# MITIBMxGraph/SALIENT_plusplus

Hardware: AMD Instinct MI355X
Metric: sampled_edges_per_sec (higher is better)
Workload: dtype int64/fp16-copy

## Files before the change

### include/spp.h

```cpp
#ifndef SPP_H
#define SPP_H

#include <stddef.h>
#include <stdint.h>

#ifdef __cplusplus
extern "C" {
#endif

#define SPP_ABI_VERSION 6
#define SPP_MAX_HOPS 8
#define SPP_MAX_PARTS 64

typedef int spp_status;
enum {
  SPP_OK = 0,
  SPP_ERR_INVALID = -1,
  SPP_ERR_HIP = -2,
  SPP_ERR_CAPACITY = -3,
  SPP_ERR_STATE = -4
};

int spp_abi_version(void);
const char* spp_last_error(void);
// ... 426 lines not shown
  int32_t reserved2;
  uint64_t seed;
} spp_agg_bwd_desc;

spp_status spp_agg_forward(const spp_agg_fwd_desc* desc, void* stream);
spp_status spp_agg_backward(const spp_agg_bwd_desc* desc, void* workspace_dev, int64_t workspace_bytes, void* stream);

spp_status spp_gather_rows_fp8(const void* q_dev, int64_t src_rows, int64_t F, const int8_t* scale_log2_dev,
                               const int64_t* idx_dev, int64_t n, void* dst_dev, void* stream);
spp_status spp_agg_forward_fp8(const spp_agg_fwd_desc* desc, const int8_t* scale_log2_dev, void* stream);

typedef struct spp_graph_agg_desc {
  int32_t epilogue;
  int32_t x_elem;
  int32_t out_elem;
  int32_t reserved;
  const int64_t* rowptr_dev;
  const int64_t* col_dev;
  const void* x_dev;
  int64_t x_stride_elems;
  int64_t x_rows;
  int64_t F;
  int64_t target_row0;
  const int64_t* target_ids_dev;
  int64_t num_targets;
  void* out_dev;
  int64_t out_stride_elems;
  float self_scale;
  int32_t reserved2;
} spp_graph_agg_desc;

int64_t spp_graph_agg_chunk(void);
int64_t spp_graph_agg_workspace_bytes(int64_t num_targets);
spp_status spp_graph_agg_forward(const spp_graph_agg_desc* desc, void* workspace_dev, int64_t workspace_bytes,
                                 void* stream);

#define SPP_GRAPH_AGG_MAX_PARTS 16
typedef struct spp_graph_agg_parts_desc {
  int32_t epilogue;
  int32_t x_elem;
  int32_t out_elem;
  int32_t num_parts;
  const int64_t* rowptr_dev;
  const int64_t* col_dev;
  int64_t part_offsets[SPP_GRAPH_AGG_MAX_PARTS + 1];
  const void* x_parts_dev[SPP_GRAPH_AGG_MAX_PARTS];
  int64_t x_stride_elems;
  int64_t F;
  int64_t target_row0;
  const int64_t* target_ids_dev;
  int64_t num_targets;
  void* out_dev;
  int64_t out_stride_elems;
  float self_scale;
  int32_t reserved;
} spp_graph_agg_parts_desc;

spp_status spp_graph_agg_parts_forward(const spp_graph_agg_parts_desc* desc, void* workspace_dev,
                                       int64_t workspace_bytes, void* stream);

typedef struct spp_graph_gat_desc {
  int32_t x_elem;
  int32_t out_elem;
  int32_t heads;
  int32_t relu;
  const int64_t* rowptr_dev;
  const int64_t* col_dev;
  const void* x_dev;
  int64_t x_stride_elems;
  int64_t x_rows;
  int64_t F;
  const float* a_src_dev;
  const float* a_dst_dev;
  int64_t target_row0;
  const int64_t* target_ids_dev;
  int64_t num_targets;
  void* out_dev;
  int64_t out_stride_elems;
  float negative_slope;
  int32_t reserved;
} spp_graph_gat_desc;

int64_t spp_graph_gat_chunk(void);
int64_t spp_graph_gat_workspace_bytes(int64_t num_targets);
spp_status spp_graph_gat_forward(const spp_graph_gat_desc* desc, void* workspace_dev, int64_t workspace_bytes,
                                 void* stream);

typedef struct spp_graph_gat_parts_desc {
  int32_t x_elem;
  int32_t out_elem;
  int32_t heads;
  int32_t relu;
  int32_t num_parts;
  int32_t reserved;
  const int64_t* rowptr_dev;
  const int64_t* col_dev;
  int64_t part_offsets[SPP_GRAPH_AGG_MAX_PARTS + 1];
  const void* h_parts_dev[SPP_GRAPH_AGG_MAX_PARTS];
  const float* a_parts_dev[SPP_GRAPH_AGG_MAX_PARTS];
  int64_t x_stride_elems;
  int64_t a_stride_elems;
  int64_t F;
  int64_t target_row0;
  const int64_t* target_ids_dev;
  int64_t num_targets;
  void* out_dev;
  int64_t out_stride_elems;
  float negative_slope;
  int32_t reserved2;
} spp_graph_gat_parts_desc;

spp_status spp_graph_gat_parts_forward(const spp_graph_gat_parts_desc* desc, void* workspace_dev,
                                       int64_t workspace_bytes, void* stream);

typedef struct spp_resinc_epilogue_desc {
  int32_t z_elem;
  int32_t r_elem;
  int32_t out_elem;
  float negative_slope;
  const void* z_dev;
  int64_t z_stride_elems;
  const float* a_dev;
  const float* b_dev;
  const void* r_dev;
  int64_t r_stride_elems;
  int64_t r_rows;
  int64_t r_row0;
  const int64_t* r_ids_dev;
  int64_t n;
  int64_t C;
  void* out_dev;
  int64_t out_stride_elems;
} spp_resinc_epilogue_desc;

spp_status spp_resinc_epilogue(const spp_resinc_epilogue_desc* desc, void* stream);

typedef struct spp_classify_desc {
  int32_t z_elem;
  int32_t reserved;
  const void* z_dev;
  int64_t z_stride_elems;
  int64_t n;
  int64_t C;
  const int64_t* y_dev;
  int64_t y_rows;
  int64_t y_row0;
  const int64_t* row_ids_dev;
  int64_t* pred_dev;
  float* nll_dev;
} spp_classify_desc;

spp_status spp_classify_rows(const spp_classify_desc* desc, void* stream);

#ifdef __cplusplus
}
#endif
#endif
```

### salient_plusplus_amd/_native.py

```python
import ctypes as C
import os

_HERE = os.path.dirname(os.path.abspath(__file__))
LIB_PATH = os.path.join(_HERE, "libspp_hip.so")

SPP_MAX_HOPS = 8
SPP_MAX_PARTS = 64

p = C.c_void_p
i32 = C.c_int32
i64 = C.c_int64
u32 = C.c_uint32


class PartitionCfg(C.Structure):
    _fields_ = [("num_parts", i32), ("rank", i32), ("offsets", i64 * (SPP_MAX_PARTS + 1)),
                ("use_cache", i32), ("cache_map_dev", p), ("cache_map_len", i64)]


class SamplerOpts(C.Structure):
    _fields_ = [("col32", i32), ("deg_tags", i32), ("row_stubs", i32), ("rng_arena", i32), ("rng_arena_mb", i64),
                ("fuse_scatter", i32), ("flag_tiled", i32), ("rows_coalesced", i32), ("dedup_preread", i32),
                ("fuse_max_edges", i64), ("initial_edge_cap", i64), ("reserved", i64 * 4)]


class SamplerCfg(C.Structure):
    _fields_ = [("rowptr_dev", p), ("col_dev", p), ("num_nodes", i64), ("nnz", i64),
                ("num_hops", i32), ("sizes", i64 * SPP_MAX_HOPS), ("max_batch", i64),
                ("num_slots", i32), ("device", i32), ("replace", i32), ("part", PartitionCfg),
                ("graph_generation", i64), ("opts", SamplerOpts)]


class SamplerInfo(C.Structure):
    _fields_ = [("col32", i32), ("deg_tags", i32), ("row_stubs", i32), ("rng_arena", i32), ("idbits", i32),
                ("tag_cap", i32), ("num_hops", i32), ("dedup_buckets_log2", i32), ("dedup_table_slots", i32),
                ("generic", i32 * SPP_MAX_HOPS), ("fused_pick", i32 * SPP_MAX_HOPS), ("flag_tiled", i32 * SPP_MAX_HOPS),
                ("rows_coalesced", i32 * SPP_MAX_HOPS), ("bucket_log2", i32 * SPP_MAX_HOPS),
                ("col32_ms", C.c_double), ("row_stubs_ms", C.c_double), ("rng_arena_ms", C.c_double),
                ("col32_bytes", i64), ("row_stubs_bytes", i64), ("rng_arena_bytes", i64), ("rng_arena_batches", i64)]


class MfgCounts(C.Structure):
    _fields_ = [("num_nodes", i64), ("num_seeds", i64), ("num_hops", i32),
                ("T", i64 * SPP_MAX_HOPS), ("S", i64 * SPP_MAX_HOPS), ("E", i64 * SPP_MAX_HOPS),
                ("draws", i64), ("part_counts", i64 * (SPP_MAX_PARTS + 2))]


class MfgOut(C.Structure):
    _fields_ = [("n_id", p), ("rowptr", p * SPP_MAX_HOPS), ("col", p * SPP_MAX_HOPS),
                ("parts", p), ("cached", p), ("perm", p), ("row_addr", p), ("x_remote", p)]


SPP_ELEM_F32, SPP_ELEM_F16, SPP_ELEM_BF16 = 0, 1, 2
SPP_ELEM_FP8_E4M3 = 3
SPP_AGG_DENSE, SPP_AGG_TABLE, SPP_AGG_ROWS = 0, 1, 2
SPP_AGG_MEAN, SPP_AGG_OPERAND, SPP_AGG_OPERAND_ACT, SPP_AGG_SUM = 0, 1, 2, 3
SPP_AGG_SCATTER, SPP_AGG_GATHER = 0, 1


class AggFwdDesc(C.Structure):
    _fields_ = [("source", i32), ("epilogue", i32), ("x_elem", i32), ("out_elem", i32), ("rowptr_dev", p),
                ("col_dev", p), ("num_targets", i64), ("x_dev", p), ("x_stride_elems", i64), ("x_rows", i64),
                ("n_id_dev", p), ("F", i64), ("out_dev", p), ("out_stride_elems", i64), ("self_scale", C.c_float),
                ("p", C.c_float), ("training", i32), ("reserved", i32), ("seed", C.c_uint64)]


class AggBwdDesc(C.Structure):
    _fields_ = [("form", i32), ("epilogue", i32), ("grad_elem", i32), ("out_elem", i32), ("z_elem", i32),
                ("reserved", i32), ("rowptr_dev", p), ("col_dev", p), ("num_targets", i64), ("num_sources", i64),
                ("num_edges", i64), ("grad_out_dev", p), ("grad_out_stride_elems", i64), ("F", i64),
                ("grad_x_dev", p), ("z_dev", p), ("self_scale", C.c_float), ("p", C.c_float), ("training", i32),
                ("reserved2", i32), ("seed", C.c_uint64)]


class GraphAggDesc(C.Structure):
    _fields_ = [("epilogue", i32), ("x_elem", i32), ("out_elem", i32), ("reserved", i32), ("rowptr_dev", p),
                ("col_dev", p), ("x_dev", p), ("x_stride_elems", i64), ("x_rows", i64), ("F", i64),
                ("target_row0", i64), ("target_ids_dev", p), ("num_targets", i64), ("out_dev", p),
                ("out_stride_elems", i64), ("self_scale", C.c_float), ("reserved2", i32)]


SPP_GRAPH_AGG_MAX_PARTS = 16


class GraphAggPartsDesc(C.Structure):
    _fields_ = [("epilogue", i32), ("x_elem", i32), ("out_elem", i32), ("num_parts", i32), ("rowptr_dev", p),
                ("col_dev", p), ("part_offsets", i64 * (SPP_GRAPH_AGG_MAX_PARTS + 1)),
                ("x_parts_dev", p * SPP_GRAPH_AGG_MAX_PARTS), ("x_stride_elems", i64), ("F", i64), ("target_row0", i64),
                ("target_ids_dev", p), ("num_targets", i64), ("out_dev", p), ("out_stride_elems", i64),
                ("self_scale", C.c_float), ("reserved", i32)]


class GraphGatDesc(C.Structure):
    _fields_ = [("x_elem", i32), ("out_elem", i32), ("heads", i32), ("relu", i32), ("rowptr_dev", p), ("col_dev", p),
                ("x_dev", p), ("x_stride_elems", i64), ("x_rows", i64), ("F", i64), ("a_src_dev", p), ("a_dst_dev", p),
                ("target_row0", i64), ("target_ids_dev", p), ("num_targets", i64), ("out_dev", p),
                ("out_stride_elems", i64), ("negative_slope", C.c_float), ("reserved", i32)]


class GraphGatPartsDesc(C.Structure):
    _fields_ = [("x_elem", i32), ("out_elem", i32), ("heads", i32), ("relu", i32), ("num_parts", i32), ("reserved", i32),
                ("rowptr_dev", p), ("col_dev", p), ("part_offsets", i64 * (SPP_GRAPH_AGG_MAX_PARTS + 1)),
                ("h_parts_dev", p * SPP_GRAPH_AGG_MAX_PARTS), ("a_parts_dev", p * SPP_GRAPH_AGG_MAX_PARTS),
                ("x_stride_elems", i64), ("a_stride_elems", i64), ("F", i64), ("target_row0", i64), ("target_ids_dev", p),
                ("num_targets", i64), ("out_dev", p), ("out_stride_elems", i64), ("negative_slope", C.c_float),
                ("reserved2", i32)]


class ResincEpilogueDesc(C.Structure):
    _fields_ = [("z_elem", i32), ("r_elem", i32), ("out_elem", i32), ("negative_slope", C.c_float), ("z_dev", p),
                ("z_stride_elems", i64), ("a_dev", p), ("b_dev", p), ("r_dev", p), ("r_stride_elems", i64),
                ("r_rows", i64), ("r_row0", i64), ("r_ids_dev", p), ("n", i64), ("C", i64), ("out_dev", p),
                ("out_stride_elems", i64)]


class ClassifyDesc(C.Structure):
    _fields_ = [("z_elem", i32), ("reserved", i32), ("z_dev", p), ("z_stride_elems", i64), ("n", i64), ("C", i64),
                ("y_dev", p), ("y_rows", i64), ("y_row0", i64), ("row_ids_dev", p), ("pred_dev", p), ("nll_dev", p)]


class GroupOut(C.Structure):
    _fields_ = [("mfg", MfgOut), ("x_out", p), ("y_out", p)]


class ExchangeCfg(C.Structure):
    _fields_ = [("comm", p), ("x_local_dev", p), ("x_local_rows", i64), ("row_bytes", i64),
                ("cache_feats_dev", p), ("cache_rows", i64), ("x_local_stride_bytes", i64),
                ("cache_stride_bytes", i64), ("peer_x_dev", C.POINTER(p)), ("peer_x_stride_bytes", i64),
                ("issue_on_consumer", i32),
                ("x_elem", i32), ("scale_log2_dev", p), ("scales_tag", C.c_uint64)]


class SessionCfg(C.Structure):
    _fields_ = [("rowptr_dev", p), ("col_dev", p), ("num_nodes", i64), ("nnz", i64),
                ("idx_dev", p), ("n_idx", i64), ("batch_size", i64), ("num_hops", i32),
                ("sizes", i64 * SPP_MAX_HOPS), ("skip_nonfull_batch", i32),
                ("force_exact_num_batches", i32), ("exact_num_batches", i64),
                ("max_items_in_queue", i32), ("group_size", i32), ("device", i32), ("sampler", p),
                ("part", C.POINTER(PartitionCfg)), ("exchange", C.POINTER(ExchangeCfg)),
                ("input_stream", p), ("order_after_input_stream", i32)]


class BatchDesc(C.Structure):
    _fields_ = [("batch_index", i64), ("start", i32), ("stop", i32), ("slot", i32),
                ("counts", MfgCounts)]


SIGNATURES = {
    "spp_abi_version": (C.c_int, []),
    "spp_last_error": (C.c_char_p, []),
    "spp_device_count": (C.c_int, []),
    "spp_async_errors": (C.c_int, [C.c_int, C.c_int]),
    "spp_profile_enable": (None, [C.c_int]),
    "spp_tune": (C.c_int, [C.c_char_p, C.c_int]),
    "spp_profile_read": (C.c_int, [C.c_int, C.POINTER(C.c_double), C.POINTER(i64), C.POINTER(i64)]),
    "spp_mt19937_fill": (C.c_int, [u32, i64, i64, p, p]),
    "spp_batch_seed": (u32, [i32]),
    "spp_gather_rows": (C.c_int, [p, i64, i64, p, C.c_int, i64, i64, p, p]),
    "spp_gather_rows_strided": (C.c_int, [p, i64, i64, i64, p, C.c_int, i64, i64, p, p]),
    "spp_to_row_major": (C.c_int, [p, i64, i64, C.c_int, p, p]),
    "spp_sampler_create": (C.c_int, [C.POINTER(SamplerCfg), C.POINTER(p)]),
    "spp_sampler_destroy": (None, [p]),
    "spp_sampler_workspace_bytes": (i64, [p]),
    "spp_sampler_deliver_stream": (p, [p]),
    "spp_sampler_get_cfg": (C.c_int, [p, C.POINTER(SamplerCfg)]),
    "spp_sampler_get_info": (C.c_int, [p, C.POINTER(SamplerInfo)]),
    "spp_sampler_sample": (C.c_int, [p, i32, p, i64, u32, i64, p]),
    "spp_sampler_wait": (C.c_int, [p, i32, C.POINTER(MfgCounts)]),
    "spp_sampler_export": (C.c_int, [p, i32, C.POINTER(MfgOut), p]),
    "spp_sampler_gather": (C.c_int, [p, i32, p, i64, i64, i64, i64, p, p]),
    "spp_nid2partid": (C.c_int, [p, i32, p, i64, p, p]),
    "spp_cache_build_map": (C.c_int, [p, i64, p, i64, p]),
    "spp_cache_lookup": (C.c_int, [p, i64, p, i64, p, p, p]),
    "spp_partition_workspace_bytes": (i64, [i64]),
    "spp_partition_batch": (C.c_int, [p, i64, p, i32, i32, i32, p, i64, i64, p, p, p, p, p, p, i64, p]),
    "spp_assemble_features": (C.c_int, [p, p, i64, p, i32, i32, i64, p, i64, p, p, p, i64, i64, i64, p, p, p]),
    "spp_session_create": (C.c_int, [C.POINTER(SessionCfg), C.POINTER(p)]),
    "spp_session_destroy": (None, [p]),
    "spp_session_num_total_batches": (i64, [p]),
    "spp_session_num_consumed_batches": (i64, [p]),
    "spp_session_batch_ranges": (C.c_int, [p, p]),
    "spp_session_next": (C.c_int, [p, C.POINTER(BatchDesc)]),
    "spp_session_export": (C.c_int, [p, C.POINTER(MfgOut), p, i64, i64, i64, p, p, i64, i64, p, p]),
    "spp_session_next_group": (C.c_int, [p, i32, C.POINTER(BatchDesc), C.POINTER(i32)]),
    "spp_session_export_group": (C.c_int, [p, i32, C.POINTER(GroupOut), p, i64, i64, i64, p, i64, i64, p]),
    "spp_session_blocked_us": (i64, [p]),
    "spp_session_blocked_occasions": (i64, [p]),
    "spp_session_sampler": (p, [p]),
    "spp_session_group_size": (i32, [p]),
    "spp_comm_unique_id": (C.c_int, [p]),
    "spp_comm_create": (C.c_int, [p, i32, i32, i32, C.POINTER(p)]),
    "spp_comm_create_local": (C.c_int, [i32, i32, C.POINTER(p)]),
    "spp_comm_destroy": (None, [p]),
    "spp_comm_rank": (i32, [p]),
    "spp_comm_world": (i32, [p]),
    "spp_vip_frequencies": (C.c_int, [p, p, i64, p, i64, i64, p, i32, p, p, p]),
    "spp_csr_mean_forward": (C.c_int, [p, p, i64, p, i32, i64, i64, p, i64, p]),
    "spp_csr_mean_backward": (C.c_int, [p, p, i64, p, i64, i64, p, p]),
    "spp_sage_operand_forward": (C.c_int, [p, p, i64, p, i32, i64, i64, p, i64, p]),
    "spp_sage_operand_forward_table": (C.c_int, [p, p, i64, p, i32, i64, i64, p, i64, p, i64, p]),
    "spp_sage_operand_backward": (C.c_int, [p, p, i64, i64, p, i64, i64, p, p]),
    "spp_sage_operand_backward_workspace_bytes": (i64, [i64, i64, i64]),
    "spp_sage_operand_backward_gather": (C.c_int, [p, p, i64, i64, i64, p, i64, i64, p, p, i64, p]),
    "spp_relu_dropout_forward": (C.c_int, [p, i64, C.c_float, i32, C.c_uint64, p, p]),
    "spp_relu_dropout_backward": (C.c_int, [p, p, i64, C.c_float, p, p]),
    "spp_sage_operand_forward_act": (C.c_int, [p, p, i64, p, i64, p, i64, C.c_float, i32, C.c_uint64, p]),
    "spp_relu_dropout_backward_pre": (C.c_int, [p, p, i64, C.c_float, i32, C.c_uint64, p, p]),
    "spp_sage_operand_backward_gather_act": (C.c_int, [p, p, i64, i64, i64, p, i64, i64, p, p, i64, p, C.c_float, i32,
                                                       C.c_uint64, p]),
    "spp_gat_forward": (C.c_int, [p, p, i64, p, i64, p, p, C.c_float, p, p, p, p]),
    "spp_gat_logits": (C.c_int, [p, i32, i64, i64, i64, i64, p, p, p, p, p]),
    "spp_gat_logits_backward": (C.c_int, [p, i32, i64, i64, i64, i64, p, p, p, p, p]),
    "spp_gat_aggregate_forward": (C.c_int, [p, p, i64, p, i32, i64, i64, p, p, C.c_float, p, p, p, p]),
    "spp_gat_aggregate_backward": (C.c_int, [p, p, i64, p, i32, i64, i64, p, p, C.c_float, p, p, p, p, p, p, p, p]),
    "spp_gat_backward": (C.c_int, [p, p, i64, p, i64, p, p, C.c_float, p, p, p, p, p, p, p, p]),
    "spp_gat_aggregate_backward_gather_workspace_bytes": (i64, [i64, i64, i64]),
    "spp_gat_aggregate_backward_gather": (C.c_int, [p, p, i64, i64, i64, p, i32, i64, i64, p, p, C.c_float, p, p, p, p,
                                                    p, p, p, p, p, p, i64, p]),
    "spp_gat_mh_logits": (C.c_int, [p, i32, i64, i64, i64, i64, i32, p, p, p, p, p]),
    "spp_gat_mh_logits_backward": (C.c_int, [p, i32, i64, i64, i64, i64, i32, p, p, p, p, p]),
    "spp_gat_mh_aggregate_forward": (C.c_int, [p, p, i64, p, i32, i64, i64, i32, p, p, C.c_float, p, p, p, p]),
    "spp_gat_mh_aggregate_backward": (C.c_int, [p, p, i64, p, i32, i64, i64, i32, p, p, C.c_float, p, p, p, p, p, p,
                                                p, p]),
    "spp_gat_mh_aggregate_backward_gather_workspace_bytes": (i64, [i64, i64, i64, i32]),
    "spp_gat_mh_aggregate_backward_gather": (C.c_int, [p, p, i64, i64, i64, p, i32, i64, i64, i32, p, p, C.c_float, p,
                                                       p, p, p, p, p, p, p, p, p, i64, p]),
    "spp_sage_operand_forward_rows": (C.c_int, [p, p, i64, p, i32, i64, p, i64, p]),
    "spp_gather_row_refs": (C.c_int, [p, i64, i64, p, p]),
    "spp_ipc_export": (C.c_int, [p, p, C.POINTER(i64)]),
    "spp_ipc_open": (C.c_int, [p, i32, C.POINTER(p)]),
    "spp_ipc_close": (C.c_int, [p]),
    "spp_csr_sum_forward": (C.c_int, [p, p, i64, p, i32, i64, i64, C.c_float, p, i64, p]),
    "spp_csr_sum_forward_table": (C.c_int, [p, p, i64, p, i32, i64, i64, p, i64, C.c_float, p, i64, p]),
    "spp_csr_sum_forward_rows": (C.c_int, [p, p, i64, p, i32, i64, C.c_float, p, i64, p]),
    "spp_csr_sum_backward": (C.c_int, [p, p, i64, i64, p, i64, i64, C.c_float, p, p]),
    "spp_csr_sum_backward_gather": (C.c_int, [p, p, i64, i64, i64, p, i64, i64, C.c_float, p, p, i64, p]),
    "spp_session_try_next": (C.c_int, [p, C.POINTER(BatchDesc)]),
    "spp_session_quiesce": (C.c_int, [p]),
    "spp_session_exchange_stats": (C.c_int, [p, C.POINTER(i64), C.POINTER(i64)]),
    "spp_agg_forward": (C.c_int, [C.POINTER(AggFwdDesc), p]),
    "spp_agg_backward": (C.c_int, [C.POINTER(AggBwdDesc), p, i64, p]),
    "spp_gather_rows_fp8": (C.c_int, [p, i64, i64, p, p, i64, p, p]),
    "spp_agg_forward_fp8": (C.c_int, [C.POINTER(AggFwdDesc), p, p]),
    "spp_graph_agg_chunk": (i64, []),
    "spp_graph_agg_workspace_bytes": (i64, [i64]),
    "spp_graph_agg_forward": (C.c_int, [C.POINTER(GraphAggDesc), p, i64, p]),
    "spp_graph_agg_parts_forward": (C.c_int, [C.POINTER(GraphAggPartsDesc), p, i64, p]),
    "spp_graph_gat_chunk": (i64, []),
    "spp_graph_gat_workspace_bytes": (i64, [i64]),
    "spp_graph_gat_forward": (C.c_int, [C.POINTER(GraphGatDesc), p, i64, p]),
    "spp_graph_gat_parts_forward": (C.c_int, [C.POINTER(GraphGatPartsDesc), p, i64, p]),
    "spp_resinc_epilogue": (C.c_int, [C.POINTER(ResincEpilogueDesc), p]),
    "spp_classify_rows": (C.c_int, [C.POINTER(ClassifyDesc), p]),
}
SPP_COMM_ID_BYTES = 128
SPP_IPC_HANDLE_BYTES = 64

_lib = None


class SppError(RuntimeError):
    pass


def load():
    global _lib
    if _lib is None:
        if not os.path.exists(LIB_PATH):
            raise SppError(
                f"{LIB_PATH} is missing: build it with `python -m salient_plusplus_amd.build` "
                "(hipcc --offload-arch=gfx950). There is no CPU fallback.")
        import torch
        L = C.CDLL(LIB_PATH)
        for name, (res, args) in SIGNATURES.items():
            fn = getattr(L, name)
            fn.restype = res
            fn.argtypes = args
        if L.spp_abi_version() != 6:
            raise SppError("libspp_hip.so ABI version mismatch")
        _lib = L
    return _lib


def check(rc: int):
    if rc < 0:
        msg = load().spp_last_error()
        raise SppError(msg.decode() if msg else f"libspp_hip error {rc}")
    return rc


def require_device():
    n = load().spp_device_count()
    if n <= 0:
        msg = load().spp_last_error()
        raise SppError("no usable HIP device for the MI355X data path: "
                       + (msg.decode() if msg else "device count 0"))
    return n
```

### salient_plusplus_amd/build.py

```python
import os
import subprocess
import sys
from concurrent.futures import ThreadPoolExecutor

HERE = os.path.dirname(os.path.abspath(__file__))
ROOT = os.path.dirname(HERE)
CSRC = os.path.join(HERE, "csrc")
OBJ = os.path.join(CSRC, "build")
LIB = os.path.join(HERE, "libspp_hip.so")
SOURCES = ["api.hip", "mt19937.hip", "gather.hip", "gather_fp8.hip", "sampler.hip", "partition.hip", "session.hip", "exchange.hip", "vip.hip", "aggregate.hip",
           "graph_aggregate.hip", "graph_gat.hip", "resinc_epilogue.hip", "classify.hip"]
HIPCC = os.environ.get("HIPCC", "/opt/rocm/bin/hipcc")
FLAGS = ["--offload-arch=gfx950", "-O3", "-std=c++17", "-fPIC", "-I" + os.path.join(ROOT, "include"),
         "-I" + CSRC, "-Wall", "-Wno-unused-function"] + os.environ.get("SPP_EXTRA_FLAGS", "").split()


def _stale(target, deps):
    if not os.path.exists(target):
        return True
    t = os.path.getmtime(target)
    return any(os.path.getmtime(d) > t for d in deps)


def build(force: bool = False, verbose: bool = False) -> str:
    os.makedirs(OBJ, exist_ok=True)
    stamp = os.path.join(OBJ, "flags.stamp")
    flags_now = " ".join([HIPCC] + FLAGS)
    if not os.path.exists(stamp) or open(stamp).read() != flags_now:
        force = True
    headers = [os.path.join(CSRC, f) for f in sorted(os.listdir(CSRC)) if f.endswith(".h")]
    headers += [os.path.join(ROOT, "include", "spp.h"), os.path.abspath(__file__)]
    jobs = []
    for src in SOURCES:
        s = os.path.join(CSRC, src)
        o = os.path.join(OBJ, src.replace(".hip", ".o"))
        if force or _stale(o, [s] + headers):
            jobs.append([HIPCC] + FLAGS + ["-c", s, "-o", o])

    def run(cmd):
        if verbose:
            print(" ".join(cmd), flush=True)
        subprocess.check_call(cmd)

    with ThreadPoolExecutor(max_workers=min(6, max(1, len(jobs)))) as ex:
        list(ex.map(run, jobs))
    objs = [os.path.join(OBJ, s.replace(".hip", ".o")) for s in SOURCES]
    if force or jobs or _stale(LIB, objs):
        run([HIPCC, "--offload-arch=gfx950", "-shared", "-fPIC", "-pthread", "-o", LIB] + objs + ["-ldl"])
    with open(stamp, "w") as f:
        f.write(flags_now)
    return LIB


if __name__ == "__main__":
    print(build(force="--force" in sys.argv, verbose=True))
```

### salient_plusplus_amd/models.py

```python
import contextlib
import ctypes as C

import torch
import torch.nn.functional as F

from . import _native as nat
from .fast_sampler import RowRefs, TableRows
from .fp8 import Fp8Features


def _p(t):
    return C.c_void_p(t.data_ptr()) if t is not None and t.numel() > 0 else None


def _stream():
    return C.c_void_p(torch._C._cuda_getCurrentRawStream(torch.cuda.current_device()))


_ELEM = {torch.float32: nat.SPP_ELEM_F32, torch.float16: nat.SPP_ELEM_F16, torch.bfloat16: nat.SPP_ELEM_BF16}


def amp_bf16():
    return torch.is_autocast_enabled("cuda") and torch.get_autocast_dtype("cuda") == torch.bfloat16

# ... 141 lines not shown

def relu_dropout(x, p=0.5, training=True):
    if x.is_cuda and x.dtype == torch.float32 and x.numel() > 0 and x.data_ptr() % 16 == 0:
        return _ReluDropout.apply(x, p, training)
    return F.dropout(F.relu(x), p=p, training=training)


def mean_aggregate(x, rowptr, col, num_targets):
    return _MeanAggregate.apply(x, rowptr, col, num_targets, False)


class _TallLinear(torch.autograd.Function):

    @staticmethod
    def forward(ctx, a, w):
        ctx.amp = amp_bf16()
        with _no_autocast():
            if ctx.amp:
                ctx.dtypes = (a.dtype, w.dtype)
                a, w = a.to(torch.bfloat16), w.to(torch.bfloat16)
            ctx.save_for_backward(a, w)
            return a @ w.t()

    @staticmethod
    def backward(ctx, g):
        a, w = ctx.saved_tensors
        if ctx.amp:
            g = g.to(torch.bfloat16).contiguous()
            grad_a = (g @ w).to(ctx.dtypes[0]) if ctx.needs_input_grad[0] else None
            grad_w = _wgrad(g, a).to(ctx.dtypes[1]) if ctx.needs_input_grad[1] else None
            return grad_a, grad_w
        grad_a = g @ w if ctx.needs_input_grad[0] else None
        grad_w = None
        if ctx.needs_input_grad[1]:
            T = a.size(0)
            slabs = min(64, T // 4096)
            if slabs >= 2 and a.is_contiguous() and g.is_contiguous():
                c = T // slabs
                head = torch.bmm(g[:slabs * c].view(slabs, c, -1).transpose(1, 2), a[:slabs * c].view(slabs, c, -1))
                grad_w = head.sum(0)
                if slabs * c < T:
                    grad_w = grad_w + g[slabs * c:].t() @ a[slabs * c:]
            else:
                grad_w = g.t() @ a
        return grad_a, grad_w


def init_weights(m):
    if isinstance(m, torch.nn.Linear):
        torch.nn.init.xavier_uniform_(m.weight, gain=torch.nn.init.calculate_gain("relu"))


class SAGEConv(torch.nn.Module):

    def __init__(self, in_channels, out_channels, bias=True):
        super().__init__()
        self.lin_l = torch.nn.Linear(in_channels, out_channels, bias=bias)
        self.lin_r = torch.nn.Linear(in_channels, out_channels, bias=False)

    def reset_parameters(self):
        self.lin_l.reset_parameters()
        self.lin_r.reset_parameters()

    def forward(self, x_pair, adj_t):
        x, x_target = x_pair
        rowptr, col, _ = adj_t.csr()
        if _is_fp8(x):
            if x_target is not None and x_target is not x:
                raise RuntimeError("SAGEConv over fp8 rows: the targets are the first rows of x (pass (x, None))")
            fused = _MeanAggregate.apply(x, rowptr, col, int(adj_t.sparse_sizes()[0]), True)
            out = _TallLinear.apply(fused, torch.cat([self.lin_l.weight, self.lin_r.weight], dim=1))
            return out if self.lin_l.bias is None else out + self.lin_l.bias
        T = x_target.size(0)
        if x_target.data_ptr() == x.data_ptr() and x_target.size(1) == x.size(1) and x_target.stride() == x.stride():
            fused = _MeanAggregate.apply(x, rowptr, col, T, True)
        else:
            mean = _MeanAggregate.apply(x, rowptr, col, T, False)
            fused = torch.cat([mean, x_target.to(mean.dtype)], dim=1)
        out = _TallLinear.apply(fused, torch.cat([self.lin_l.weight, self.lin_r.weight], dim=1))
        return out if self.lin_l.bias is None else out + self.lin_l.bias


class SAGE(torch.nn.Module):
    def __init__(self, in_channels, hidden_channels, out_channels, num_layers):
        super().__init__()
        self.num_layers = num_layers
        self.hidden_channels = hidden_channels
        self.convs = torch.nn.ModuleList()
        self.convs.append(SAGEConv(in_channels, hidden_channels, bias=False))
        for _ in range(num_layers - 2):
            self.convs.append(SAGEConv(hidden_channels, hidden_channels, bias=False))
        self.convs.append(SAGEConv(hidden_channels, out_channels, bias=False))
        self.reset_parameters()

    def reset_parameters(self):
        for conv in self.convs:
            conv.reset_parameters()
            conv.apply(init_weights)

    def forward(self, x, adjs):
        if x.is_cuda and _SageStack.usable(self, x, adjs):
            hops = []
            for adj_t, _e_id, size in adjs:
                rowptr, col, _ = adj_t.csr()
                hops.append((rowptr, col, int(size[1])))
            weights = [w for conv in self.convs for w in (conv.lin_l.weight, conv.lin_r.weight)]
            if isinstance(x, TableRows):
                x = (x.table, x.n_id)
            elif isinstance(x, RowRefs):
                x = _Refs(x)
            return _SageStack.apply(x, hops, self.training, 0.5, *weights)
        if isinstance(x, (TableRows, RowRefs)):
            x = x.materialize()
        elif isinstance(x, Fp8Features):
            x = x.dequantize(torch.float16)
        for i, (adj_t, _e_id, size) in enumerate(adjs):
            x_target = x[:size[1]]
            x = self.convs[i]((x, x_target), adj_t)
            if i != self.num_layers - 1:
                x = relu_dropout(x, 0.5, self.training)
        return torch.log_softmax(x, dim=-1)

    @torch.no_grad()
    def inference(self, x_all, rowptr, col, **kw):
        from .inference import layerwise_inference
        return layerwise_inference(self, x_all, rowptr, col, **kw)


def _wgrad(g, a):
    T = a.size(0)
    slabs = min(64, T // 2048)
    if slabs < 2:
        return (g.t() @ a).float()
    c = T // slabs
    acc = torch.bmm(a[:slabs * c].view(slabs, c, -1).transpose(1, 2), g[:slabs * c].view(slabs, c, -1)).sum(
        0, dtype=torch.float32)
    if slabs * c < T:
        if g.dtype == torch.float32:
            acc.addmm_(a[slabs * c:].t(), g[slabs * c:])
        else:
            acc.add_(a[slabs * c:].t() @ g[slabs * c:])
    return acc.t()


def _split_wgrad(gW):
    N, K2 = gW.shape
    base = gW.t()
    if not base.is_contiguous():
        return gW[:, :K2 // 2].contiguous(), gW[:, K2 // 2:].contiguous()
    both = base.view(2, K2 // 2, N).transpose(1, 2).contiguous()
    return both[0], both[1]


def _tall_linear(a, w):
    return torch.nn.functional.linear(a, w)


def _readable(x):
    if isinstance(x, RowRefs):
        return x.dtype in _ELEM
    m = x.table if isinstance(x, TableRows) else x
    if isinstance(m, Fp8Features):
        return m.is_cuda
    return m.is_cuda and m.dim() == 2 and m.stride(1) == 1 and m.dtype in _ELEM


class _SageStack(torch.autograd.Function):

    @staticmethod
    def usable(model, x, adjs):
        rows = x.table if isinstance(x, TableRows) else x
        if not _readable(x) or (isinstance(rows, torch.Tensor) and rows.requires_grad):
            return False
        k = x.size(1)
        for conv in model.convs:
            if conv.lin_l.bias is not None or conv.lin_l.weight.dtype != torch.float32 or k % 4:
                return False
            k = conv.lin_l.weight.size(0)
        return len(adjs) == len(model.convs)

    @staticmethod
    def forward(ctx, x, hops, training, p, *weights):
        if _is_fp8(x):
            _no_input_grad(ctx, "SAGE")
        nat.require_device()
        ctx.amp = amp_bf16()
        dt = torch.bfloat16 if ctx.amp else torch.float32
        st = _stream()
        n_layers = len(hops)
        operands, acts, wcats, seeds = [], [], [], []
        with _no_autocast():
            for i, (rowptr, col, T) in enumerate(hops):
                if i == 0:
                    A = _agg_forward(nat.SPP_AGG_OPERAND, rowptr, col, T, x, dt, st=st)
                else:
                    A = _agg_forward(nat.SPP_AGG_OPERAND_ACT, rowptr, col, T, Z, dt, act=(p, bool(training), seeds[i - 1]),
                                     st=st)
                wl, wr = weights[2 * i], weights[2 * i + 1]
                W = torch.cat([wl, wr], dim=1, out=torch.empty((wl.size(0), A.size(1)), dtype=dt, device=A.device))
                Z = _tall_linear(A, W)
                operands.append(A)
                wcats.append(W)
                if i != n_layers - 1:
                    seeds.append(int(torch.empty((), dtype=torch.int64).random_().item()) if training else 0)
                    acts.append(Z)
            out = torch.log_softmax(Z, dim=-1, dtype=torch.float32)
        hop_t = [t for (rowptr, col, _T) in hops for t in (rowptr, col)]
        ctx.save_for_backward(*operands, *acts, *wcats, out, *hop_t)
        ctx.hop_T = [int(T) for (_r, _c, T) in hops]
        ctx.act = (float(p), int(bool(training)), seeds)
        batch_rows = x[1].numel() if isinstance(x, tuple) else x.r.size(0) if isinstance(x, _Refs) else x.size(0)
        ctx.src_rows = [batch_rows] + [a.size(0) for a in acts]
        return out

    @staticmethod
    @torch.autograd.function.once_differentiable
    def backward(ctx, g_out):
        st = _stream()
        dt = torch.bfloat16 if ctx.amp else torch.float32
        n_layers = len(ctx.hop_T)
        sv = ctx.saved_tensors
        operands, acts = sv[:n_layers], sv[n_layers:2 * n_layers - 1]
        wcats, out = sv[2 * n_layers - 1:3 * n_layers - 1], sv[3 * n_layers - 1]
        hop_t = sv[3 * n_layers:]
        hops = [(hop_t[2 * i], hop_t[2 * i + 1], ctx.hop_T[i]) for i in range(n_layers)]
        p_, training_, seeds = ctx.act
        grads = [None] * (2 * n_layers)
        with _no_autocast():
            gZ = torch._log_softmax_backward_data(g_out.float().contiguous(), out, -1, torch.float32).to(dt)
            for i in range(n_layers - 1, -1, -1):
                A, W = operands[i], wcats[i]
                K = A.size(1) // 2
                gW = _wgrad(gZ, A)
                grads[2 * i], grads[2 * i + 1] = _split_wgrad(gW)
                if i == 0:
                    break
                rowptr, col, T = hops[i]
                gA = gZ @ W
                gZ = _agg_backward(nat.SPP_AGG_OPERAND_ACT, rowptr, col, T, ctx.src_rows[i], gA, K, dt,
                                   gather=col.numel() * K >= (1 << 22), z=acts[i - 1],
                                   act=(p_, training_, seeds[i - 1]), st=st)
        return (None, None, None, None, *grads)


class _GatAggregate(torch.autograd.Function):

    @staticmethod
    def forward(ctx, h, a_src, a_dst, rowptr, col, slope):
        L = nat.load()
        nat.require_device()
        h, a_src, a_dst = h.contiguous().float(), a_src.contiguous().float(), a_dst.contiguous().float()
        T, Fdim = a_dst.numel(), h.size(1)
        out = torch.empty((T, Fdim), dtype=torch.float32, device=h.device)
        rmax = torch.empty(T, dtype=torch.float32, device=h.device)
        rsum = torch.empty(T, dtype=torch.float32, device=h.device)
        nat.check(L.spp_gat_forward(_p(rowptr), _p(col), T, _p(h), Fdim, _p(a_src), _p(a_dst), float(slope), _p(out),
                                    _p(rmax), _p(rsum), _stream()))
        ctx.save_for_backward(h, a_src, a_dst, rowptr, col, out, rmax, rsum)
        ctx.slope = float(slope)
        return out

    @staticmethod
    def backward(ctx, g):
        h, a_src, a_dst, rowptr, col, out, rmax, rsum = ctx.saved_tensors
        T, Fdim = a_dst.numel(), h.size(1)
        g = g.contiguous().float()
        grad_h = torch.zeros_like(h)
        grad_as = torch.zeros_like(a_src)
        grad_ad = torch.zeros_like(a_dst)
        nat.check(nat.load().spp_gat_backward(_p(rowptr), _p(col), T, _p(h), Fdim, _p(a_src), _p(a_dst), ctx.slope,
                                              _p(out), _p(rmax), _p(rsum), _p(g), _p(grad_h), _p(grad_as), _p(grad_ad),
                                              _stream()))
        return grad_h, grad_as, grad_ad, None, None, None


class GATConv(torch.nn.Module):

    def __init__(self, in_channels, out_channels, heads=1, concat=True, negative_slope=0.2, bias=True):
        super().__init__()
        if not isinstance(heads, int) or heads < 1:
            raise ValueError(f"heads must be a positive int, got {heads!r}")
        self.heads, self.out_channels, self.concat = heads, out_channels, bool(concat)
        self.negative_slope = negative_slope
        self.lin_src = torch.nn.Linear(in_channels, heads * out_channels, bias=False)
        self.lin_dst = self.lin_src
        self.att_src = torch.nn.Parameter(torch.empty(1, heads, out_channels))
        self.att_dst = torch.nn.Parameter(torch.empty(1, heads, out_channels))
        width = heads * out_channels if concat else out_channels
        self.bias = torch.nn.Parameter(torch.zeros(width)) if bias else None
        self.reset_parameters()

    def reset_parameters(self):
        self.lin_src.reset_parameters()
        torch.nn.init.xavier_uniform_(self.att_src)
        torch.nn.init.xavier_uniform_(self.att_dst)
        if self.bias is not None:
            torch.nn.init.zeros_(self.bias)

    def forward(self, x_pair, adj_t):
        if self.heads != 1:
            return self._forward_heads(x_pair, adj_t)
        x, x_target = x_pair
        rowptr, col, _ = adj_t.csr()
        T, K = x_target.size(0), x.size(1)
        if (x.is_cuda and x.dim() == 2 and x.stride(1) == 1 and x.dtype in _ELEM and
                K % 4 == 0 and K <= 1024 and x_target.data_ptr() == x.data_ptr() and x_target.stride() == x.stride()):
            out = _GatLayer.apply(x, self.lin_src.weight, self.att_src.view(-1), self.att_dst.view(-1), rowptr, col, T,
                                  self.negative_slope)
            return out if self.bias is None else out + self.bias
        h = _TallLinear.apply(x.to(torch.float32), self.lin_src.weight)
        h_t = h[:x_target.size(0)]
        a_src = (h * self.att_src.view(1, -1)).sum(-1)
        a_dst = (h_t * self.att_dst.view(1, -1)).sum(-1)
        out = _GatAggregate.apply(h, a_src, a_dst, rowptr, col, self.negative_slope)
        return out if self.bias is None else out + self.bias

    def _forward_heads(self, x_pair, adj_t):
        x, x_target = x_pair
        rowptr, col, _ = adj_t.csr()
        T, K, H = x_target.size(0), x.size(1), self.heads
        att_src, att_dst = self.att_src.view(H, -1), self.att_dst.view(H, -1)
        if (H in _GAT_MH_HEADS and x.is_cuda and x.dim() == 2 and x.stride(1) == 1 and x.dtype in _ELEM and
                K % 4 == 0 and K <= 1024 and x_target.data_ptr() == x.data_ptr() and x_target.stride() == x.stride()):
            out = _GatLayerMH.apply(x, self.lin_src.weight, att_src, att_dst, rowptr, col, T, self.negative_slope,
                                    self.concat)
        else:
            out = _gat_mh_reference(x, x_target, self.lin_src.weight, att_src, att_dst, rowptr, col,
                                    self.negative_slope, self.concat)
        return out if self.bias is None else out + self.bias


_GAT_MH_HEADS = (1, 2, 4, 8)


def _gat_mh_reference(x, x_target, W, att_src, att_dst, rowptr, col, slope, concat):
    H, Cc = att_src.shape
    S, T = x.size(0), x_target.size(0)
    h = F.linear(x.to(W.dtype), W).view(S, H, Cc)
    h_t = h[:T] if x_target.data_ptr() == x.data_ptr() and x_target.stride() == x.stride() else \
        F.linear(x_target.to(W.dtype), W).view(T, H, Cc)
    a_src = (h * att_src).sum(-1)
    a_dst = (h_t * att_dst).sum(-1)
    dst = torch.repeat_interleave(torch.arange(T, device=col.device), rowptr[1:] - rowptr[:-1])
    keep = col != dst
    loops = torch.arange(T, device=col.device)
    src, dst = torch.cat([col[keep], loops]), torch.cat([dst[keep], loops])
    e = F.leaky_relu(a_src[src].float() + a_dst[dst].float(), slope)
    emax = torch.full((T, H), float("-inf"), device=e.device).scatter_reduce(0, dst[:, None].expand(-1, H), e, "amax")
    w = torch.exp(e - emax[dst])
    den = torch.zeros((T, H), device=e.device).index_add_(0, dst, w)
    alpha = w / den[dst]
    out = torch.zeros((T, H, Cc), device=e.device).index_add_(0, dst, alpha[:, :, None] * h[src].float())
    return out.reshape(T, H * Cc) if concat else out.mean(1)


class _GatLayerMH(torch.autograd.Function):

    @staticmethod
    def forward(ctx, x, W, att_src, att_dst, rowptr, col, T, slope, concat):
        ctx.amp = amp_bf16()
        with _no_autocast():
            return _GatLayerMH._forward(ctx, x, W, att_src, att_dst, rowptr, col, T, slope, concat)

    @staticmethod
    def _forward(ctx, x, W, att_src, att_dst, rowptr, col, T, slope, concat):
        L = nat.load()
        nat.require_device()
        st = _stream()
        S, K = x.size(0), x.size(1)
        H, Cc = att_src.shape
        elem = _ELEM[x.dtype]
        xs = x.stride(0) if S > 1 else K
        W3 = W.to(torch.float32).view(H, Cc, K)
        att = torch.stack([att_src, att_dst]).to(torch.float32)
        V = torch.einsum("shc,hck->shk", att, W3).contiguous()
        f32 = dict(dtype=torch.float32, device=x.device)
        a_src, a_dst = torch.empty((S, H), **f32), torch.empty((T, H), **f32)
        nat.check(L.spp_gat_mh_logits(_p(x), elem, xs, S, T, K, H, _p(V[0]), _p(V[1]), _p(a_src), _p(a_dst), st))
        z = torch.empty((T, H, K), **f32)
        rmax, rsum = torch.empty((T, H), **f32), torch.empty((T, H), **f32)
        nat.check(L.spp_gat_mh_aggregate_forward(_p(rowptr), _p(col), T, _p(x), elem, xs, K, H, _p(a_src), _p(a_dst),
                                                 float(slope), _p(z), _p(rmax), _p(rsum), st))
        ctx.save_for_backward(x, W, att_src, att_dst, rowptr, col, a_src, a_dst, z, rmax, rsum, V)
        ctx.dims = (S, T, K, H, Cc, elem, xs, float(slope), bool(concat))
        dt = torch.bfloat16 if ctx.amp else torch.float32
        zc, Wc = z.to(dt), W.to(dt).view(H, Cc, K)
        if concat:
# ... 405 lines not shown
```

Baseline: 8.686 billion.

## Add split-K weight-gradient reduction kernel and fused multi-layer weight packing

Replaces the per-layer torch.cat weight concatenation with a single native kernel that packs all layers' [wl|wr] weights into one buffer, cast to the compute dtype. In backward, the weight gradient is now computed as a batched split-K matmul over row slabs. A custom kernel then sums the slabs, transposes the result and writes the two halves straight into the wl/wr gradient buffers, replacing the previous wgrad plus split path. This cuts kernel launches and small copies per step, at the cost of extra memory for the partial products and new alignment and shape edge cases.

```diff
diff --git a/include/spp.h b/include/spp.h
--- a/include/spp.h
+++ b/include/spp.h
@@ -602,6 +602,25 @@
 
 spp_status spp_classify_rows(const spp_classify_desc* desc, void* stream);
 
+#define SPP_PACK_MAX_LAYERS 8
+
+typedef struct spp_pack_weights_desc {
+  int32_t num_layers;
+  int32_t out_elem;
+  const float* w_l_dev[SPP_PACK_MAX_LAYERS];
+  const float* w_r_dev[SPP_PACK_MAX_LAYERS];
+  int64_t N[SPP_PACK_MAX_LAYERS];
+  int64_t K[SPP_PACK_MAX_LAYERS];
+  int64_t out_offset_elems[SPP_PACK_MAX_LAYERS];
+  void* out_dev;
+  int64_t out_elems;
+} spp_pack_weights_desc;
+
+spp_status spp_wgrad_reduce_split(const void* partials_dev, int64_t partials_elems, int32_t elem, int64_t slabs,
+                                  const void* tail_dev, int64_t K, int64_t N, float* grad_wl_dev, float* grad_wr_dev,
+                                  void* stream);
+spp_status spp_pack_weights(const spp_pack_weights_desc* desc, void* stream);
+
 #ifdef __cplusplus
 }
 #endif
diff --git a/salient_plusplus_amd/_native.py b/salient_plusplus_amd/_native.py
--- a/salient_plusplus_amd/_native.py
+++ b/salient_plusplus_amd/_native.py
@@ -117,6 +117,15 @@
 class ClassifyDesc(C.Structure):
     _fields_ = [("z_elem", i32), ("reserved", i32), ("z_dev", p), ("z_stride_elems", i64), ("n", i64), ("C", i64),
                 ("y_dev", p), ("y_rows", i64), ("y_row0", i64), ("row_ids_dev", p), ("pred_dev", p), ("nll_dev", p)]
+
+
+SPP_PACK_MAX_LAYERS = 8
+
+
+class PackWeightsDesc(C.Structure):
+    _fields_ = [("num_layers", i32), ("out_elem", i32), ("w_l_dev", p * SPP_PACK_MAX_LAYERS),
+                ("w_r_dev", p * SPP_PACK_MAX_LAYERS), ("N", i64 * SPP_PACK_MAX_LAYERS), ("K", i64 * SPP_PACK_MAX_LAYERS),
+                ("out_offset_elems", i64 * SPP_PACK_MAX_LAYERS), ("out_dev", p), ("out_elems", i64)]
 
 
 class GroupOut(C.Structure):
@@ -252,6 +261,8 @@
     "spp_graph_gat_parts_forward": (C.c_int, [C.POINTER(GraphGatPartsDesc), p, i64, p]),
     "spp_resinc_epilogue": (C.c_int, [C.POINTER(ResincEpilogueDesc), p]),
     "spp_classify_rows": (C.c_int, [C.POINTER(ClassifyDesc), p]),
+    "spp_wgrad_reduce_split": (C.c_int, [p, i64, i32, i64, p, i64, i64, p, p, p]),
+    "spp_pack_weights": (C.c_int, [C.POINTER(PackWeightsDesc), p]),
 }
 SPP_COMM_ID_BYTES = 128
 SPP_IPC_HANDLE_BYTES = 64
diff --git a/salient_plusplus_amd/build.py b/salient_plusplus_amd/build.py
--- a/salient_plusplus_amd/build.py
+++ b/salient_plusplus_amd/build.py
@@ -9,7 +9,7 @@
 OBJ = os.path.join(CSRC, "build")
 LIB = os.path.join(HERE, "libspp_hip.so")
 SOURCES = ["api.hip", "mt19937.hip", "gather.hip", "gather_fp8.hip", "sampler.hip", "partition.hip", "session.hip", "exchange.hip", "vip.hip", "aggregate.hip",
-           "graph_aggregate.hip", "graph_gat.hip", "resinc_epilogue.hip", "classify.hip"]
+           "graph_aggregate.hip", "graph_gat.hip", "resinc_epilogue.hip", "classify.hip", "step_glue.hip"]
 HIPCC = os.environ.get("HIPCC", "/opt/rocm/bin/hipcc")
 FLAGS = ["--offload-arch=gfx950", "-O3", "-std=c++17", "-fPIC", "-I" + os.path.join(ROOT, "include"),
          "-I" + CSRC, "-Wall", "-Wno-unused-function"] + os.environ.get("SPP_EXTRA_FLAGS", "").split()
diff --git a/salient_plusplus_amd/csrc/step_glue.hip b/salient_plusplus_amd/csrc/step_glue.hip
--- /dev/null
+++ b/salient_plusplus_amd/csrc/step_glue.hip
@@ -0,0 +1,180 @@
+#include "elem_io.hip.h"
+
+namespace spp {
+
+constexpr int kWgNT = 256, kTile = 32, kDepth = 16;
+
+template <typename Tp, bool VEC4>
+__device__ __forceinline__ f4 wg_load(const Tp* p, int64_t cols_left) {
+  if constexpr (VEC4) {
+    return load4(p);
+  } else {
+    f4 v = {0.f, 0.f, 0.f, 0.f};
+    if (cols_left > 0) v.x = load1(p);
+    if (cols_left > 1) v.y = load1(p + 1);
+    if (cols_left > 2) v.z = load1(p + 2);
+    if (cols_left > 3) v.w = load1(p + 3);
+    return v;
+  }
+}
+
+template <typename Tp, bool VEC4>
+__global__ __launch_bounds__(kWgNT) void k_wgrad_reduce_split(const Tp* __restrict__ part, int64_t slabs,
+                                                              const Tp* __restrict__ tail, int64_t K, int64_t N,
+                                                              float* __restrict__ gl, float* __restrict__ gr) {
+  __shared__ float tile[kTile][kTile + 1];
+  const int64_t n0 = (int64_t)blockIdx.x * kTile, k0 = (int64_t)blockIdx.y * kTile;
+  const int r = threadIdx.x >> 3, c = threadIdx.x & 7;
+  const int64_t k = k0 + r, n = n0 + 4 * c;
+  f4 acc = {0.f, 0.f, 0.f, 0.f};
+  if (k < 2 * K && n < N) {
+    const int64_t left = N - n, slab = 2 * K * N;
+    const Tp* p = part + k * N + n;
+    auto add = [&](f4 v) { acc.x += v.x; acc.y += v.y; acc.z += v.z; acc.w += v.w; };
+    int64_t s = 0;
+    for (; s + kDepth <= slabs; s += kDepth) {
+      f4 v[kDepth];
+#pragma unroll
+      for (int u = 0; u < kDepth; ++u) v[u] = wg_load<Tp, VEC4>(p + (s + u) * slab, left);
+#pragma unroll
+      for (int u = 0; u < kDepth; ++u) add(v[u]);
+    }
+    for (; s + 4 <= slabs; s += 4) {
+      f4 v[4];
+#pragma unroll
+      for (int u = 0; u < 4; ++u) v[u] = wg_load<Tp, VEC4>(p + (s + u) * slab, left);
+#pragma unroll
+      for (int u = 0; u < 4; ++u) add(v[u]);
+    }
+    for (; s < slabs; ++s) add(wg_load<Tp, VEC4>(p + s * slab, left));
+    if (tail) add(wg_load<Tp, VEC4>(tail + k * N + n, left));
+  }
+  tile[4 * c + 0][r] = acc.x;
+  tile[4 * c + 1][r] = acc.y;
+  tile[4 * c + 2][r] = acc.z;
+  tile[4 * c + 3][r] = acc.w;
+  __syncthreads();
+  const int kk = threadIdx.x & (kTile - 1);
+  const int64_t ko = k0 + kk;
+  if (ko >= 2 * K) return;
+  float* dst = ko < K ? gl + ko : gr + (ko - K);
+#pragma unroll
+  for (int nn = threadIdx.x / kTile; nn < kTile; nn += kWgNT / kTile)
+    if (n0 + nn < N) dst[(n0 + nn) * K] = tile[nn][kk];
+}
+
+constexpr int kPackNT = 256, kPackSpan = 4 * kPackNT;
+
+struct PackTable {
+  const float* wl[SPP_PACK_MAX_LAYERS];
+  const float* wr[SPP_PACK_MAX_LAYERS];
+  int64_t K[SPP_PACK_MAX_LAYERS];
+  int64_t elems[SPP_PACK_MAX_LAYERS];
+  int64_t offset[SPP_PACK_MAX_LAYERS];
+  uint32_t block0[SPP_PACK_MAX_LAYERS];
+};
+
+template <typename Tout, bool VEC4>
+__global__ __launch_bounds__(kPackNT) void k_pack_weights(PackTable t, Tout* __restrict__ out) {
+  const uint32_t b = blockIdx.x;
+  const float *wl = t.wl[0], *wr = t.wr[0];
+  int64_t K = t.K[0], elems = t.elems[0], off = t.offset[0];
+  uint32_t b0 = 0;
+#pragma unroll
+  for (int l = 1; l < SPP_PACK_MAX_LAYERS; ++l)
+    if (b >= t.block0[l]) {
+      wl = t.wl[l], wr = t.wr[l], K = t.K[l], elems = t.elems[l], off = t.offset[l], b0 = t.block0[l];
+    }
+  const int64_t e = (int64_t)(b - b0) * kPackSpan + 4 * (int64_t)threadIdx.x;
+  if (e >= elems) return;
+  const int64_t row = e / (2 * K), col = e - row * 2 * K;
+  if constexpr (VEC4) {
+    const float* src = col < K ? wl + row * K + col : wr + row * K + (col - K);
+    store4(out + off + e, load4(src));
+  } else {
+#pragma unroll
+    for (int u = 0; u < 4; ++u) {
+      const int64_t eu = e + u;
+      if (eu >= elems) break;
+      const int64_t ru = eu / (2 * K), cu = eu - ru * 2 * K;
+      store1(out + off + eu, cu < K ? wl[ru * K + cu] : wr[ru * K + (cu - K)]);
+    }
+  }
+}
+
+}
+
+using namespace spp;
+
+extern "C" spp_status spp_wgrad_reduce_split(const void* partials_dev, int64_t partials_elems, int32_t elem,
+                                             int64_t slabs, const void* tail_dev, int64_t K, int64_t N,
+                                             float* grad_wl_dev, float* grad_wr_dev, void* stream) {
+  const char* who = "spp_wgrad_reduce_split";
+  SPP_REQUIRE(f32_bf16_ok(elem), "%s: unknown or unsupported element code %d", who, (int)elem);
+  SPP_REQUIRE(slabs >= 1 && K >= 1 && N >= 1, "%s: slabs, K and N must be positive", who);
+  SPP_REQUIRE(K < (1ll << 30) && N < (1ll << 31) && slabs < (1ll << 31) && ceil_div(2 * K, kTile) <= 65535,
+              "%s: sizes out of range", who);
+  SPP_REQUIRE(partials_dev && grad_wl_dev && grad_wr_dev, "%s: NULL buffer", who);
+  SPP_REQUIRE(partials_elems / (2 * K) / N >= slabs, "%s: the partial products hold fewer than slabs * 2K * N elements",
+              who);
+  SPP_REQUIRE(aligned_to(partials_dev, elem_bytes(elem)) && (!tail_dev || aligned_to(tail_dev, elem_bytes(elem))) &&
+                  aligned_to(grad_wl_dev, 4) && aligned_to(grad_wr_dev, 4),
+              "%s: buffers must be aligned to their element", who);
+  const int64_t vb = 4 * elem_bytes(elem);
+  const bool vec = N % 4 == 0 && aligned_to(partials_dev, vb) && (!tail_dev || aligned_to(tail_dev, vb));
+  const dim3 grid((unsigned)ceil_div(N, kTile), (unsigned)ceil_div(2 * K, kTile));
+  with_f32_bf16(elem, [&](auto tp) {
+    using Tp = typename decltype(tp)::type;
+    auto launch = [&](auto v) {
+      hipLaunchKernelGGL((k_wgrad_reduce_split<Tp, decltype(v)::value>), grid, dim3(kWgNT), 0, as_stream(stream),
+                         static_cast<const Tp*>(partials_dev), slabs, static_cast<const Tp*>(tail_dev), K, N,
+                         grad_wl_dev, grad_wr_dev);
+    };
+    vec ? launch(std::true_type{}) : launch(std::false_type{});
+  });
+  SPP_HIP_TRY(hipGetLastError());
+  return SPP_OK;
+}
+
+extern "C" spp_status spp_pack_weights(const spp_pack_weights_desc* desc, void* stream) {
+  const char* who = "spp_pack_weights";
+  SPP_REQUIRE(desc, "%s: NULL descriptor", who);
+  const spp_pack_weights_desc& d = *desc;
+  SPP_REQUIRE(d.num_layers >= 0 && d.num_layers <= SPP_PACK_MAX_LAYERS, "%s: %d layers (at most %d)", who,
+              (int)d.num_layers, SPP_PACK_MAX_LAYERS);
+  SPP_REQUIRE(f32_bf16_ok(d.out_elem), "%s: unknown or unsupported element code %d", who, (int)d.out_elem);
+  if (d.num_layers == 0) return SPP_OK;
+  const int64_t eb = elem_bytes(d.out_elem);
+  SPP_REQUIRE(d.out_dev && aligned_to(d.out_dev, 16), "%s: NULL or unaligned output", who);
+  PackTable t{};
+  bool vec = true;
+  int64_t blocks = 0;
+  for (int l = 0; l < SPP_PACK_MAX_LAYERS; ++l) {
+    t.block0[l] = 0xffffffffu;
+    if (l >= d.num_layers) continue;
+    const int64_t N = d.N[l], K = d.K[l];
+    SPP_REQUIRE(N >= 1 && K >= 1 && N < (1ll << 31) && K < (1ll << 30), "%s: layer %d: bad shape", who, l);
+    SPP_REQUIRE(d.w_l_dev[l] && d.w_r_dev[l] && aligned_to(d.w_l_dev[l], 4) && aligned_to(d.w_r_dev[l], 4),
+                "%s: layer %d: NULL or unaligned weight", who, l);
+    const int64_t elems = 2 * N * K, off = d.out_offset_elems[l];
+    SPP_REQUIRE(off >= 0 && (off * eb) % 16 == 0, "%s: layer %d: the offset is not 16-byte aligned", who, l);
+    SPP_REQUIRE(off + elems <= d.out_elems, "%s: layer %d: the output is too small", who, l);
+    for (int m = 0; m < l; ++m)
+      SPP_REQUIRE(off >= t.offset[m] + t.elems[m] || off + elems <= t.offset[m], "%s: layers %d and %d overlap", who, m, l);
+    vec = vec && K % 4 == 0 && aligned_to(d.w_l_dev[l], 16) && aligned_to(d.w_r_dev[l], 16);
+    t.wl[l] = d.w_l_dev[l], t.wr[l] = d.w_r_dev[l], t.K[l] = K, t.elems[l] = elems, t.offset[l] = off;
+    t.block0[l] = (uint32_t)blocks;
+    blocks += ceil_div(elems, kPackSpan);
+    SPP_REQUIRE(blocks < (1ll << 31), "%s: too many elements", who);
+  }
+  with_f32_bf16(d.out_elem, [&](auto to) {
+    using Tout = typename decltype(to)::type;
+    auto launch = [&](auto v) {
+      hipLaunchKernelGGL((k_pack_weights<Tout, decltype(v)::value>), dim3((unsigned)blocks), dim3(kPackNT), 0,
+                         as_stream(stream), t, static_cast<Tout*>(d.out_dev));
+    };
+    vec ? launch(std::true_type{}) : launch(std::false_type{});
+  });
+  SPP_HIP_TRY(hipGetLastError());
+  return SPP_OK;
+}
diff --git a/salient_plusplus_amd/models.py b/salient_plusplus_amd/models.py
--- a/salient_plusplus_amd/models.py
+++ b/salient_plusplus_amd/models.py
@@ -317,6 +317,44 @@
     return both[0], both[1]
 
 
+def _wgrad_split(g, a):
+    T, K2 = a.shape
+    N = g.size(1)
+    slabs = min(64, T // 2048)
+    tail = None
+    if slabs < 2:
+        slabs, part = 1, a.t() @ g
+    else:
+        c = T // slabs
+        part = torch.bmm(a[:slabs * c].view(slabs, c, -1).transpose(1, 2), g[:slabs * c].view(slabs, c, -1))
+        if slabs * c < T:
+            tail = a[slabs * c:].t() @ g[slabs * c:]
+    both = torch.empty((2, N, K2 // 2), dtype=torch.float32, device=a.device)
+    nat.check(nat.load().spp_wgrad_reduce_split(_p(part), part.numel(), _ELEM[part.dtype], slabs, _p(tail), K2 // 2, N,
+                                                _p(both[0]), _p(both[1]), _stream()))
+    return both[0], both[1]
+
+
+def _pack_weights(weights, dt):
+    pairs = [(weights[2 * i], weights[2 * i + 1]) for i in range(len(weights) // 2)]
+    if len(pairs) > nat.SPP_PACK_MAX_LAYERS or not all(
+            w.is_contiguous() and w.dtype == torch.float32 and w.numel() > 0 for pr in pairs for w in pr):
+        return [torch.cat([wl, wr], dim=1, out=torch.empty((wl.size(0), 2 * wl.size(1)), dtype=dt, device=wl.device))
+                for wl, wr in pairs]
+    d = nat.PackWeightsDesc(num_layers=len(pairs), out_elem=_ELEM[dt])
+    total = 0
+    for i, (wl, wr) in enumerate(pairs):
+        d.w_l_dev[i], d.w_r_dev[i] = wl.data_ptr(), wr.data_ptr()
+        d.N[i], d.K[i] = wl.shape
+        d.out_offset_elems[i] = total
+        total += -(-2 * wl.numel() // 128) * 128
+    out = torch.empty(total, dtype=dt, device=pairs[0][0].device)
+    d.out_dev, d.out_elems = out.data_ptr(), total
+    nat.check(nat.load().spp_pack_weights(C.byref(d), _stream()))
+    return [out[d.out_offset_elems[i]:d.out_offset_elems[i] + 2 * wl.numel()].view(wl.size(0), 2 * wl.size(1))
+            for i, (wl, _wr) in enumerate(pairs)]
+
+
 def _tall_linear(a, w):
     return torch.nn.functional.linear(a, w)
 
@@ -353,19 +391,17 @@
         dt = torch.bfloat16 if ctx.amp else torch.float32
         st = _stream()
         n_layers = len(hops)
-        operands, acts, wcats, seeds = [], [], [], []
+        operands, acts, seeds = [], [], []
         with _no_autocast():
+            wcats = _pack_weights(weights, dt)
             for i, (rowptr, col, T) in enumerate(hops):
                 if i == 0:
                     A = _agg_forward(nat.SPP_AGG_OPERAND, rowptr, col, T, x, dt, st=st)
                 else:
                     A = _agg_forward(nat.SPP_AGG_OPERAND_ACT, rowptr, col, T, Z, dt, act=(p, bool(training), seeds[i - 1]),
                                      st=st)
-                wl, wr = weights[2 * i], weights[2 * i + 1]
-                W = torch.cat([wl, wr], dim=1, out=torch.empty((wl.size(0), A.size(1)), dtype=dt, device=A.device))
-                Z = _tall_linear(A, W)
+                Z = _tall_linear(A, wcats[i])
                 operands.append(A)
-                wcats.append(W)
                 if i != n_layers - 1:
                     seeds.append(int(torch.empty((), dtype=torch.int64).random_().item()) if training else 0)
                     acts.append(Z)
@@ -396,8 +432,7 @@
             for i in range(n_layers - 1, -1, -1):
                 A, W = operands[i], wcats[i]
                 K = A.size(1) // 2
-                gW = _wgrad(gZ, A)
-                grads[2 * i], grads[2 * i + 1] = _split_wgrad(gW)
+                grads[2 * i], grads[2 * i + 1] = _wgrad_split(gZ, A)
                 if i == 0:
                     break
                 rowptr, col, T = hops[i]
```

After: 8.664 billion, median of 2. About the same (-0.3%).
